# GLAD-RUC/FastEGNN

Measured on NVIDIA B200. Metric: layer fwd+bwd edges/sec (full train step: fwd+MSE+MMD+bwd+Adam), Water-3D shape, higher is better.
Workload: dtype tf32: tcgen05 TF32 operand tiles with fp32 accumulation and tanh.approx SiLU in the edge and virtual phases (fp16 operands with power-of-two scales in the edge backward), TF32 tiles in the node-side backward, error-compensated 3xTF32 tiles (fp32-grade) in the node-side forward, fp32 FMA in the per-g

## Files before the change

### fastegnn_b200/csrc/api.cu

```cuda
#include <cstdarg>
#include <cstdio>
#include <cstdlib>
#include <cstring>

#include "common.cuh"
#include "adam.cu"
#include "edge_kernels.cu"
#include "edge_tc.cu"
#include "edge_tc_bwd.cu"
#include "edge_tc_bwd2.cu"
#include "edge_tc_bwd3.cu"
#include "edge_tc_bwd4.cu"
#include "graph_kernels.cu"
#include "graph_prep.cu"
#include "radius_graph.cu"
#include "halo.cu"
#include "mmd.cu"
#include "node_kernels.cu"
#include "virtual_kernels.cu"
#include "virtual_tc.cu"
#include "node_tc.cu"
#include "dense_tc.cu"
#include "segment.cu"
#include "peak_probe.cu"
// ... 29 lines not shown
#define TRY(expr)            \
  do {                       \
    int rc__ = (expr);       \
    if (rc__ != 0) return rc__; \
  } while (0)

int g_edge_fwd_mode = 1;
int g_edge_bwd_mode = 6;

int g_virt_fwd_mode = 1;
int g_virt_bwd_mode = 1;
int g_node_fwd_mode = 3;
const bool g_node_pre_tc3 = getenv("FEGNN_NODE_PRE_TC3") == nullptr || atoi(getenv("FEGNN_NODE_PRE_TC3")) != 0;
int g_node_bwd_mode = 2;
int g_det = 0;
constexpr int kNodeTcMinN = 0;
inline bool node_bwd_tc(int N) { return g_node_bwd_mode == 1 || (g_node_bwd_mode == 2 && N >= kNodeTcMinN); }

int sm_count() {
  static int sms[64] = {};
  int dev = 0;
  if (cudaGetDevice(&dev) != cudaSuccess || dev < 0 || dev >= 64) return 148;
  if (sms[dev] == 0) {
    if (cudaDeviceGetAttribute(&sms[dev], cudaDevAttrMultiProcessorCount, dev) != cudaSuccess || sms[dev] <= 0) sms[dev] = 148;
  }
  return sms[dev];
}

int check_loss_ws(int N, int B, const float* ws, size_t floats) {
  if (!g_det) return 0;
// ... 126 lines not shown
  atomicAdd(gvnf + k * C + c, acc);
}
__global__ void final_gx_kernel(int N, const float* __restrict__ gx, const float* __restrict__ gxsum,
                                const int* __restrict__ batch, float* __restrict__ out) {
  int idx = blockIdx.x * blockDim.x + threadIdx.x;
  if (idx >= N * 3) return;
  int i = idx / 3, k = idx - i * 3;
  out[idx] = gx[idx] + gxsum[batch[i] * 3 + k];
}

}

namespace {

struct SideStream {
  cudaStream_t st = nullptr;
  cudaEvent_t fork = nullptr, join = nullptr, aux = nullptr;
};
SideStream* side_stream() {
  static SideStream per_dev[64];
  int dev = 0;
  if (cudaGetDevice(&dev) != cudaSuccess || dev < 0 || dev >= 64) return nullptr;
  SideStream* s = &per_dev[dev];
  if (s->st == nullptr) {
    if (cudaStreamCreateWithFlags(&s->st, cudaStreamNonBlocking) != cudaSuccess) return nullptr;
    if (cudaEventCreateWithFlags(&s->fork, cudaEventDisableTiming) != cudaSuccess) return nullptr;
    if (cudaEventCreateWithFlags(&s->join, cudaEventDisableTiming) != cudaSuccess) return nullptr;
    if (cudaEventCreateWithFlags(&s->aux, cudaEventDisableTiming) != cudaSuccess) return nullptr;
  }
  return s;
}
#define FORK(side, main)                                 \
  do {                                                   \
    CK(cudaEventRecord((side)->fork, (main)));           \
    CK(cudaStreamWaitEvent((side)->st, (side)->fork, 0)); \
  } while (0)
#define JOIN(side, main)                                 \
  do {                                                   \
    CK(cudaEventRecord((side)->join, (side)->st));       \
    CK(cudaStreamWaitEvent((main), (side)->join, 0));    \
  } while (0)

}
// ... 21 lines not shown
    if (mode != 0 && mode != 1 && !(mode == 2 && !fwd) && !(mode == 3 && fwd))
      return fail(FEGNN_EINVAL, "%s mode must be 0 or 1%s", phase, fwd ? " or 3 (3xTF32 phi_h)" : " or 2 (auto)");
    (fwd ? g_node_fwd_mode : g_node_bwd_mode) = mode;
    return 0;
  }
  if (strcmp(phase, "virtual_forward") == 0 || strcmp(phase, "virtual_backward") == 0) {
    if (mode != 0 && mode != 1) return fail(FEGNN_EINVAL, "%s mode must be 0 or 1", phase);
    (phase[8] == 'f' ? g_virt_fwd_mode : g_virt_bwd_mode) = mode;
    return 0;
  }
  if (strcmp(phase, "deterministic") == 0) {
    if (mode != 0 && mode != 1) return fail(FEGNN_EINVAL, "deterministic mode must be 0 or 1");
    g_det = mode;
    return 0;
  }
  return fail(FEGNN_EINVAL, "unknown phase '%s'", phase);
}
int fegnn_get_mode(const char* phase) {
  if (phase != nullptr && strcmp(phase, "edge_forward") == 0) return g_edge_fwd_mode;
  if (phase != nullptr && strcmp(phase, "edge_backward") == 0) return g_edge_bwd_mode;
  if (phase != nullptr && strcmp(phase, "node_forward") == 0) return g_node_fwd_mode;
  if (phase != nullptr && strcmp(phase, "node_backward") == 0) return g_node_bwd_mode;
  if (phase != nullptr && strcmp(phase, "virtual_forward") == 0) return g_virt_fwd_mode;
  if (phase != nullptr && strcmp(phase, "virtual_backward") == 0) return g_virt_bwd_mode;
  if (phase != nullptr && strcmp(phase, "deterministic") == 0) return g_det;
  return -1;
}

size_t fegnn_graph_prep_workspace_bytes(int32_t N, int32_t E) { return graph_prep_workspace_bytes(N, E); }

int fegnn_graph_prep(int32_t N, int32_t E, int32_t B, int32_t Fe, const int64_t* edge_index, const int64_t* data_batch,
                     const float* edge_attr, int32_t* perm, int32_t* rowptr, int32_t* row, int32_t* col,
                     int32_t* batch, int32_t* gptr, float* edge_attr_sorted, float* dinv, float* inv_nb,
                     void* workspace, size_t workspace_bytes, void* stream) {
  RQ(N >= 0 && E >= 0 && B >= 0 && Fe >= 0);
  RQ(rowptr && gptr && (N == 0 || (batch && data_batch && dinv)) && (B == 0 || inv_nb));
  RQ(E == 0 || (edge_index && perm && row && col && workspace));
  RQ(E == 0 || Fe == 0 || (edge_attr && edge_attr_sorted));
  if (workspace_bytes < graph_prep_workspace_bytes(N, E))
    return fail(FEGNN_ENOMEM, "graph_prep workspace %zu < %zu bytes", workspace_bytes, graph_prep_workspace_bytes(N, E));
// ... 225 lines not shown
    CK(launch_dense_bwd_tc(t2, sm_count(), S(stream)));
    return 0;
  }
  CK(launch_node_h_bwd(a, sm_count(), S(stream)));
  return 0;
}

int fegnn_virtual_backward(const fegnn_dims* d, const fegnn_graph* g, const fegnn_layer_params* p,
                           fegnn_layer_grads* gr, const float* x, const float* v, const float* Z,
                           const fegnn_layer_saved* sv, const float* gx_new, const float* gxsum_next,
                           const float* gDsum, const float* gUsum, const float* gu, float* gAv, float* gG1, float* gx,
                           float* gZ, float* gsv, float* gsg, float* gt, void* stream) {
  return fegnn_virtual_backward_inputs(d, g, p, gr, x, v, Z, sv, gx_new, gxsum_next, gDsum, gUsum, gu, gAv, gG1, gx, gZ, gsv,
                                       gsg, gt, nullptr, stream);
}
int fegnn_virtual_backward_inputs(const fegnn_dims* d, const fegnn_graph* g, const fegnn_layer_params* p,
                                  fegnn_layer_grads* gr, const float* x, const float* v, const float* Z,
                                  const fegnn_layer_saved* sv, const float* gx_new, const float* gxsum_next,
                                  const float* gDsum, const float* gUsum, const float* gu, float* gAv, float* gG1, float* gx,
                                  float* gZ, float* gsv, float* gsg, float* gt, const fegnn_input_grads* ig, void* stream) {
  NO_DET("the layer kernels add edge, node and graph sums across CTAs with float atomics");
  TRY(check_dims(d));
  TRY(check_flags_params(d, p));
  TRY(check_input_grads(d, ig));
  RQ(g && gr && x && v && Z && sv && gx_new && gDsum && gAv && gG1 && gx && gZ && gsv && gt);
  RQ(!(d->flags & FEGNN_F_GRAVITY) || gsg);
  VirtArgs a = virt_args(d, g, p, x, v, Z, sv);
  a.gx_new = gx_new; a.gxsum_next = gxsum_next; a.gDsum = gDsum; a.gUsum = gUsum; a.gu = gu;
  a.gAv = gAv; a.gG1 = gG1; a.gx = gx; a.gZ = gZ; a.gsv = gsv; a.gsg = gsg; a.gt = gt;
  a.g_wv1 = gr->edgev_w0; a.g_V2 = gr->edgev_w2; a.g_c2 = gr->edgev_b2;
  a.g_Wxv = gr->crv_w0; a.g_bxv = gr->crv_b0; a.g_wxv = gr->crv_w2;
  a.g_WX = gr->cvv_w0; a.g_bX = gr->cvv_b0; a.g_wX = gr->cvv_w2;
  a.g_wav = gr->attv_w; a.g_bav = gr->attv_b;
  if (!(d->flags & FEGNN_F_PREZEROED)) CK(zero_pair(gG1, kH * d->C * (size_t)d->B, gx, 3 * (size_t)d->Nl, S(stream)));
  if (d->flags & FEGNN_F_LAST) a.gu = nullptr;
  if (g_virt_bwd_mode == 1 && !(d->flags & FEGNN_F_ATTENTION) && gu != nullptr) {
    a.gu_work = const_cast<float*>(gu);
    a.u = sv->u;
    a.stats = reinterpret_cast<unsigned*>(sv->scratch);
    CK(launch_virtual_bwd_tc<4>(a, sm_count(), S(stream)));
  } else {
    CK(launch_virtual_bwd(a, sm_count(), S(stream)));
  }
  if (ig != nullptr && ig->node_vel != nullptr)
    CK(launch_input_grad_vel(d->N, sv->sv, gx_new, gxsum_next, g->batch, ig->node_vel, S(stream)));
  return 0;
}

int fegnn_edge_backward(const fegnn_dims* d, const fegnn_graph* g, const fegnn_layer_params* p, fegnn_layer_grads* gr,
                        const float* x, const fegnn_layer_saved* sv, const float* gm, const float* gt, float* gP,
                        float* gQ, float* gx, void* stream) {
  return fegnn_edge_backward_inputs(d, g, p, gr, x, sv, gm, gt, gP, gQ, gx, nullptr, stream);
}
int fegnn_edge_backward_inputs(const fegnn_dims* d, const fegnn_graph* g, const fegnn_layer_params* p, fegnn_layer_grads* gr,
                               const float* x, const fegnn_layer_saved* sv, const float* gm, const float* gt, float* gP,
                               float* gQ, float* gx, const fegnn_input_grads* ig, void* stream) {
  NO_DET("the layer kernels add edge, node and graph sums across CTAs with float atomics");
  TRY(check_dims(d));
  TRY(check_flags_params(d, p));
  TRY(check_input_grads(d, ig));
  RQ(g && gr && x && sv && gt && gP && gQ && gx);
  EdgeArgs a = edge_args(d, g, p, x, sv);
  a.gm = gm; a.gt = gt; a.gP = gP; a.gQ = gQ; a.gx = gx;
  a.g_w1 = gr->edge_w0; a.g_W2 = gr->edge_w2; a.g_b2 = gr->edge_b2;
  a.g_W3 = gr->cr_w0; a.g_b3 = gr->cr_b0; a.g_w4 = gr->cr_w2; a.g_wa = gr->att_w; a.g_ba = gr->att_b;
  const bool zero = !(d->flags & FEGNN_F_PREZEROED);
  if (zero) CK(zero_pair(gP, kH * (size_t)d->N, gQ, kH * (size_t)d->Nl, S(stream)));
  const bool tc_ok = d->Fe <= kTcMaxFe && !(d->flags & FEGNN_F_ATTENTION);
  int mode = g_edge_bwd_mode;
  if (mode == 6) mode = (tc_ok && sv->scratch != nullptr) ? 7 : 4;
  if ((mode == 7 || mode == 8) && (!tc_ok || sv->scratch == nullptr)) mode = 4;
  const bool pre = !(d->flags & FEGNN_F_STATS_READY);
  if (ig != nullptr && ig->edge_attr != nullptr) {
    a.g_ea = ig->edge_attr;
    a.perm = ig->perm;
    if (tc_ok && sv->scratch != nullptr && mode == 7) {
      CK((launch_edge_bwd_tc4<2, true>(a, reinterpret_cast<unsigned*>(sv->scratch), sm_count(), S(stream), zero && pre, pre)));
    } else {
      CK(launch_edge_bwd<true>(a, sm_count(), S(stream)));
    }
    return 0;
  }
  if (mode == 7) CK(launch_edge_bwd_tc4<2>(a, reinterpret_cast<unsigned*>(sv->scratch), sm_count(), S(stream), zero && pre, pre));
  else if (mode == 8) CK(launch_edge_bwd_tc4<4>(a, reinterpret_cast<unsigned*>(sv->scratch), sm_count(), S(stream), zero && pre, pre));
  else if (mode == 5 && tc_ok && sv->scratch != nullptr)
    CK(launch_edge_bwd_tc3(a, reinterpret_cast<unsigned*>(sv->scratch), sm_count(), S(stream), zero));
  else if (mode == 2 && tc_ok) CK(launch_edge_bwd_tc2<2>(a, sm_count(), S(stream)));
  else if ((mode == 4 || mode == 5) && tc_ok) CK(launch_edge_bwd_tc2<4>(a, sm_count(), S(stream)));
  else if (mode == 1 && tc_ok) CK(launch_edge_bwd_tc(a, sm_count(), S(stream)));
  else CK(launch_edge_bwd(a, sm_count(), S(stream)));
  return 0;
}

int fegnn_graph_pre_backward(const fegnn_dims* d, const fegnn_graph* g, const fegnn_layer_params* p,
                             fegnn_layer_grads* gr, const float* Sf, const fegnn_layer_saved* sv, const float* gG1,
                             float* gS, float* gZ, float* gxsum, void* stream) {
  NO_DET("the layer kernels add edge, node and graph sums across CTAs with float atomics");
  TRY(check_dims(d));
  RQ(g && p && gr && Sf && sv && gG1 && gS && gZ && gxsum);
  GraphArgs a = graph_args(d, g, p);
  a.S = Sf; a.M = sv->M; a.Zc = sv->Zc; a.gG1 = gG1; a.gS = gS; a.gZ = gZ; a.gxsum = gxsum;
  a.g_wv1 = gr->edgev_w0;
  CK(launch_graph_pre_bwd(a, S(stream)));
  return 0;
}

// ... 183 lines not shown
  const size_t N = d->N, Nl = d->Nl, B = d->B, C = d->C;
  float* p = base;
  auto take = [&](size_t n) { float* r = p; p += al4(n); return r; };
  for (int l = 0; l <= L; ++l) w->xsum[l] = take(B * 3);
  for (int l = 0; l <= L; ++l) {
    w->h[l] = take(N * kH); w->x[l] = take(Nl * 3); w->Z[l] = take(B * 3 * C); w->Sx[l] = take(B * C * kH);
  }
  for (int l = 0; l < L; ++l) {
    fegnn_layer_saved_bind(d, p, &w->saved[l]);
    p += fegnn_layer_saved_floats(d);
  }
}

struct BwdScratch {
  float *gh, *gx[2], *gZ[2], *gS[2], *gxsum[2], *gDsum, *gUsum, *gzh1, *gm, *gu, *gAv, *gG1[2], *gsv, *gsg, *gt, *gP[2], *gQ[2];
  size_t set_a_floats, set_b_floats;
};
size_t bwd_scratch_floats(const fegnn_dims* d) {
  const size_t N = d->N, Nl = d->Nl, B = d->B, C = d->C;
  return al4(N * kH) + 2 * al4(Nl * 3) + 2 * al4(B * 3 * C) + 2 * al4(B * C * kH) + 2 * al4(B * 3) + al4(B * 3 * C) +
         al4(B * C * kH) + 2 * al4(N * kH) + al4(N * C * kH) + al4(N * kH) + 2 * al4(B * C * kH) + 2 * al4(N) +
         al4(N * 3) + 2 * (al4(N * kH) + al4(Nl * kH));
}
void bwd_scratch_bind(const fegnn_dims* d, float* base, BwdScratch* s) {
  const size_t N = d->N, Nl = d->Nl, B = d->B, C = d->C;
  float* p = base;
  auto take = [&](size_t n) { float* r = p; p += al4(n); return r; };
  s->gh = take(N * kH);
  for (int k = 0; k < 2; ++k) { s->gG1[k] = take(B * C * kH); s->gx[k] = take(Nl * 3); }
  s->set_a_floats = al4(B * C * kH) + Nl * 3;
  s->gZ[0] = take(B * 3 * C); s->gZ[1] = take(B * 3 * C);
  s->gS[0] = take(B * C * kH); s->gS[1] = take(B * C * kH);
  s->gxsum[0] = take(B * 3); s->gxsum[1] = take(B * 3);
  s->gDsum = take(B * 3 * C); s->gUsum = take(B * C * kH);
  s->gzh1 = take(N * kH); s->gm = take(N * kH); s->gu = take(N * C * kH);
  s->gAv = take(N * kH);
  s->gsv = take(N); s->gsg = take(N); s->gt = take(N * 3);
  for (int k = 0; k < 2; ++k) { s->gP[k] = take(N * kH); s->gQ[k] = take(Nl * kH); }
  s->set_b_floats = al4(N * kH) + Nl * kH;
}

}

extern "C" {

size_t fegnn_model_workspace_floats(const fegnn_dims* d, int32_t L) { return model_ws_floats(d, L); }
size_t fegnn_model_backward_scratch_floats(const fegnn_dims* d) { return bwd_scratch_floats(d); }

int fegnn_model_forward(const fegnn_dims* d, int32_t L, int32_t Fin, const fegnn_graph* g,
                        const fegnn_layer_params* layers, const float* embed_w, const float* embed_b,
                        const float* vnf, const float* node_feat, const float* x0, const float* v,
                        const float* loc_mean, float* x_out, float* Z_out, float* workspace, size_t workspace_floats,
                        void* stream) {
  NO_DET("the layer kernels add edge, node and graph sums across CTAs with float atomics");
// ... 225 lines not shown
    dl.flags |= FEGNN_F_PREZEROED;
    const bool last = rf || l == L - 1;
    if (last) dl.flags |= FEGNN_F_LAST;
    const fegnn_layer_params* p = &layers[l];
    fegnn_layer_grads* gr = &grads[l];
    const fegnn_layer_saved* sv = &w.saved[l];
    const int ls = rf ? 0 : l;
    static const bool stats_fused = getenv("FEGNN_STATS_FUSED") == nullptr || atoi(getenv("FEGNN_STATS_FUSED")) != 0;
    if (stats_fused && !rf && g_virt_bwd_mode == 1 && !(d->flags & FEGNN_F_ATTENTION) && sv->scratch != nullptr &&
        (last || (node_bwd_tc(d->N) && dense_bwd_uses_rows(d->N, sm_count()))))
      dl.flags |= FEGNN_F_STATS_READY;
    TRY(fegnn_graph_post_backward(&dl, g, p, gr, w.Sx[ls], sv, gZ_new, gS_new, s.gZ[cur], s.gS[cur], s.gDsum, s.gUsum,
                                  side));
    if (!last) TRY(fegnn_node_h_backward(&dl, g, p, gr, sv, s.gh, s.gzh1, s.gm, s.gu, stream));
    JOIN(sd, st);
    TRY(fegnn_virtual_backward_inputs(&dl, g, p, gr, w.x[l], v, w.Z[l], sv, gx_new, gxsum_next, s.gDsum,
                                      last ? nullptr : s.gUsum, s.gu, s.gAv, s.gG1[cur], s.gx[cur], s.gZ[cur],
                                      s.gsv, s.gsg, s.gt, ig, stream));
    FORK(sd, st);
    TRY(fegnn_graph_pre_backward(&dl, g, p, gr, w.Sx[ls], sv, s.gG1[cur], s.gS[cur], s.gZ[cur], s.gxsum[cur], side));
    if (l > 0) {
      CK(cudaMemsetAsync(s.gG1[cur ^ 1], 0, sizeof(float) * s.set_a_floats, S(side)));
      CK(cudaMemsetAsync(s.gP[cur ^ 1], 0, sizeof(float) * s.set_b_floats, S(side)));
    }
    TRY(fegnn_edge_backward_inputs(&dl, g, p, gr, w.x[l], sv, last ? nullptr : s.gm, s.gt, s.gP[cur], s.gQ[cur], s.gx[cur],
                                   ig, stream));
    if (rf) TRY(fegnn_rf_vel_backward(d->N, v, p, gr, s.gsv, stream));
    TRY(fegnn_node_pre_backward_inputs(&dl, p, gr, w.h[ls], s.gP[cur], s.gQ[cur], s.gAv, last ? nullptr : s.gzh1, s.gsv, s.gsg,
                                       s.gh, ig, stream));
    gx_new = s.gx[cur]; gZ_new = s.gZ[cur]; gS_new = s.gS[cur]; gxsum_next = s.gxsum[cur];
    cur ^= 1;
  }
  FORK(sd, st);
  if (N > 0) {
    final_gx_kernel<<<(unsigned)((N * 3 + 255) / 256), 256, 0, S(side)>>>(d->N, gx_new, gxsum_next, g->batch, g_x0); ++g_launches;
    CK(cudaGetLastError());
  }
  CK(cudaMemcpyAsync(g_loc_mean, gZ_new, sizeof(float) * 3 * C * B, cudaMemcpyDeviceToDevice, S(side)));
  if (B > 0) {
    reduce_gS_kernel<<<(unsigned)((C * kH + 255) / 256), 256, 0, S(side)>>>(d->B, d->C, gS_new, g_vnf); ++g_launches;
    CK(cudaGetLastError());
// ... 83 lines not shown
```

### fastegnn_b200/csrc/edge_tc_bwd4.cu

```cuda
#include "common.cuh"
#include "umma.cuh"
#include <cuda_fp16.h>

namespace fegnn {
namespace bwd4 {

using bwd2::elect_one;
using bwd2::tmem_ld;
using bwd2::tmem_st_wait;
using bwd3::desc_add;
using bwd3::gemm_ts_k;
using bwd3::gemm_ts_mn;
using bwd3::gemm_wgrad;
using bwd3::h_chunk_off;
using bwd3::idesc_f16;
using bwd3::kTileBytes;
using bwd3::kWBytes;
using bwd3::make_desc_h;
using bwd3::pack2;
using bwd3::unpack2;

__device__ __forceinline__ uint32_t h2u(__half2 h) { return *reinterpret_cast<uint32_t*>(&h); }
__device__ __forceinline__ __half2 u2h(uint32_t u) { return *reinterpret_cast<__half2*>(&u); }
__device__ __forceinline__ __half2 tanh_h2(__half2 x) {
// ... 66 lines not shown
  float w4f[kH], wqf[kH];
  unsigned mw[2];
  uint32_t tmem_slot;
};
struct Geo {
  int srow[kTM], scol[kTM];
  float sq[kTM], snrm[kTM], sd[kTM * 3], sgte[kTM * 3], sgs[kTM], sea[kTM * kTcMaxFe];
};
template <int CG>
struct GroupVec {
  Geo geo[2];
  int irow[kTM], icol[kTM];
  float iea[kTM * kTcMaxFe];
  float spart[CG * kTM], sgqp[CG * kTM], ss[kTM];
  uint64_t bar[6];
};
__device__ __forceinline__ void cp_async4(void* dst, const void* src) {
  asm volatile("cp.async.ca.shared.global [%0], [%1], 4;" :: "r"(umma::smem_u32(dst)), "l"(src) : "memory");
}
__device__ __forceinline__ void cp_async_wait_all() { asm volatile("cp.async.wait_all;" ::: "memory"); }
template <int CG>
struct Smem4 {
  static constexpr int off_W2 = 0, off_W3 = kWBytes;
  static constexpr int off_groups = 2 * kWBytes;
  static constexpr int g_TA = 0, g_TM = kTileBytes, g_AUX = 2 * kTileBytes, g_TG = 3 * kTileBytes, g_T3 = 4 * kTileBytes;
  static constexpr int g_vec = 5 * kTileBytes;
  static constexpr int g_bytes = ((g_vec + (int)sizeof(GroupVec<CG>) + 1023) / 1024) * 1024;
  static constexpr int off_svec = off_groups + 2 * g_bytes;
  static constexpr size_t bytes = off_svec + sizeof(SharedVec) + 1024;
};
constexpr uint32_t kACC = 0, kOPA = 64, kD2T = 96, kD1T = 128, kGroupCols = 160;
constexpr uint32_t kR3 = 320, kR2 = 392, kDXZ = 464, kDW4 = 472;

__device__ __forceinline__ float pow2_to(float bound, int e_target) {
  if (!(bound > 0.f) || !(bound < 3.0e38f)) return 1.f;
  int e;
  frexpf(bound, &e);
  e = e_target - e;
  e = e < -60 ? -60 : (e > 60 ? 60 : e);
  return ldexpf(1.f, e);
}

template <int CG, bool kEa>
__global__ void __launch_bounds__(256 * CG, 1) edge_bwd_tc4_kernel(EdgeArgs a, const unsigned* stats) {
  VTR_DECL();
  constexpr int NTG = 128 * CG, NT = 2 * NTG, CPT = kH / CG, NP = CPT / 2, NWG = NTG / 32, RPW = kTM / NWG;
  using SM = Smem4<CG>;
  using GV = GroupVec<CG>;
  extern __shared__ uint8_t smem_raw[];
  uint8_t* smem = smem_raw + ((1024u - (umma::smem_u32(smem_raw) & 1023u)) & 1023u);
  SharedVec* sv = reinterpret_cast<SharedVec*>(smem + SM::off_svec);
  const int t = threadIdx.x, G = t / NTG, tg = t - G * NTG, wg = tg >> 5, lane = t & 31;
  const int quarter = wg & 3, cg = wg >> 2, row = quarter * 32 + lane, c0 = cg * CPT;
  uint8_t* gs = smem + SM::off_groups + G * SM::g_bytes;
  GV* v = reinterpret_cast<GV*>(gs + SM::g_vec);
  uint8_t *TA = gs + SM::g_TA, *TM = gs + SM::g_TM, *AUX = gs + SM::g_AUX, *TG = gs + SM::g_TG, *T3 = gs + SM::g_T3;
  const bool use_tanh = a.flags & FEGNN_F_TANH, norm = a.flags & FEGNN_F_NORMALIZE;
  auto group_sync = [&]() { asm volatile("bar.sync %0, %1;" :: "r"(1 + G), "n"(NTG) : "memory"); };
  pdl_trigger();
// ... 85 lines not shown
  const float k32 = s2 / s3, k21 = s1 / s2;
  const float r3 = 1.f / s3, r2 = 1.f / s2, r1 = 1.f / s1, ra = 1.f / sa, rdot = 1.f / sdot, rq = 1.f / (s1 * swq);
  const uint32_t tbase = tmem + G * kGroupCols;
  const uint32_t tlane = tbase + ((uint32_t)(quarter * 32) << 16);
  const uint32_t twg = tmem + ((uint32_t)(16 * G) << 16);
  const uint32_t id_k = idesc_f16(128, 64, 0, 0), id_mn = idesc_f16(128, 64, 0, 1);
  const uint32_t id_wg72 = idesc_f16(64, 72, 1, 1), id_aux = idesc_f16(64, 8, 1, 1);
  const uint64_t dW2k = make_desc_h(umma::smem_u32(smem + SM::off_W2), 16), dW3k = make_desc_h(umma::smem_u32(smem + SM::off_W3), 16);
  const uint64_t dW2m = make_desc_h(umma::smem_u32(smem + SM::off_W2), kWBytes), dW3m = make_desc_h(umma::smem_u32(smem + SM::off_W3), kWBytes);
  const uint64_t dTG = make_desc_h(umma::smem_u32(TG), kTileBytes);
  const uint64_t dTM_AUX = make_desc_h(umma::smem_u32(TM), kTileBytes);
  const uint64_t dTA_AUX = make_desc_h(umma::smem_u32(TA), 2 * kTileBytes);
  const uint64_t dTMa = make_desc_h(umma::smem_u32(TM), kTileBytes);
  const uint64_t dT3a = make_desc_h(umma::smem_u32(T3), kTileBytes);
  const uint64_t dAUX = make_desc_h(umma::smem_u32(AUX), kTileBytes);
  uint32_t phase = 0;
  bool first_tile = true;
  const int l16 = lane & 15, hsel = lane >> 4;

  const int ntiles = (a.E + kTM - 1) / kTM, tstride = gridDim.x * 2;
  auto load_idx_async = [&](int tl) {
    const int e = tl * kTM + tg;
    if (e < a.E) {
      cp_async4(&v->irow[tg], a.row + e);
      cp_async4(&v->icol[tg], a.col + e);
      for (int f = 0; f < a.Fe; ++f) cp_async4(&v->iea[tg * kTcMaxFe + f], a.ea + (size_t)e * a.Fe + f);
    } else {
      v->irow[tg] = -1;
    }
  };
  auto geometry = [&](Geo* gg) {
    cp_async_wait_all();
    const int r = v->irow[tg];
    int c = 0;
    float d0 = 0, d1 = 0, d2 = 0, q = 0, nrm = 1.f, g0 = 0, g1 = 0, g2 = 0;
// ... 14 lines not shown
#pragma unroll
    for (int f = 0; f < kTcMaxFe; ++f) gg->sea[tg * kTcMaxFe + f] = ea[f];
    gg->sd[tg * 3 + 0] = d0; gg->sd[tg * 3 + 1] = d1; gg->sd[tg * 3 + 2] = d2;
    if (norm) {
      nrm = sqrtf(q) + a.eps;
      const float inv = 1.f / nrm;
      d0 *= inv; d1 *= inv; d2 *= inv;
    }
    gg->srow[tg] = r;
    gg->scol[tg] = c;
    gg->sq[tg] = q;
    gg->snrm[tg] = nrm;
    gg->sgte[tg * 3 + 0] = g0; gg->sgte[tg * 3 + 1] = g1; gg->sgte[tg * 3 + 2] = g2;
    gg->sgs[tg] = d0 * g0 + d1 * g1 + d2 * g2;
  };
  int cur = 0;
  if (tg < kTM && blockIdx.x * 2 + G < ntiles) {
    load_idx_async(blockIdx.x * 2 + G);
    geometry(&v->geo[0]);
    if (blockIdx.x * 2 + G + tstride < ntiles) load_idx_async(blockIdx.x * 2 + G + tstride);
  }
  for (int tile = blockIdx.x * 2 + G; tile < ntiles; tile += tstride, cur ^= 1) {
    const Geo* geo = &v->geo[cur];
    if (!first_tile) {
      umma::mbar_wait(&v->bar[4], phase ^ 1);
    VTR();
      umma::fence_after();
    }
    umma::fence_before();
    group_sync();
    VTR();
    if (tg < kTM)
      *reinterpret_cast<uint4*>(AUX + h_chunk_off(tg, 0)) =
          make_uint4(pack2(geo->srow[tg] >= 0 ? 1.f : 0.f, geo->sq[tg]), pack2(geo->sea[tg * kTcMaxFe], geo->sea[tg * kTcMaxFe + 1]),
                     pack2(geo->sea[tg * kTcMaxFe + 2], geo->sea[tg * kTcMaxFe + 3]), 0u);
    group_sync();
    VTR();
    {
// ... 51 lines not shown
      tmem_stu<NP>(tlane + kD1T + cg * NP, pd);
      tmem_st_wait();
    }
    umma::fence_smem_to_async();
    umma::fence_before();
    group_sync();
    VTR();
    if (wg == 0) {
      umma::fence_after();
      if (elect_one()) {
        gemm_ts_k(tbase + kACC, tbase + kOPA, dW2k, id_k);
        umma::commit(&v->bar[0]);
      }
      __syncwarp();
    }
    if (tg < kTM && tile + tstride < ntiles) {
      geometry(&v->geo[cur ^ 1]);
      if (tile + 2 * tstride < ntiles) load_idx_async(tile + 2 * tstride);
    }
    umma::mbar_wait(&v->bar[0], phase);
    VTR();
    umma::fence_after();
    {
      float z[CPT];
      uint32_t pm[NP], pd[NP];
      tmem_ld<CPT>(tlane + kACC + c0, z);
#pragma unroll
      for (int j = 0; j < CPT; j += 4) {
        const float4 hb = *reinterpret_cast<const float4*>(sv->hb2 + c0 + j);
        __half2 a0, e0, a1v, e1;
        silu_grad_h2(__floats2half2_rn(fmaf(z[j], 0.5f, hb.x), fmaf(z[j + 1], 0.5f, hb.y)), a0, e0);
        silu_grad_h2(__floats2half2_rn(fmaf(z[j + 2], 0.5f, hb.z), fmaf(z[j + 3], 0.5f, hb.w)), a1v, e1);
        pm[j >> 1] = h2u(a0); pm[(j >> 1) + 1] = h2u(a1v);
// ... 172 lines not shown
        }
      }
    }
    umma::fence_smem_to_async();
    umma::fence_before();
    group_sync();
    VTR();
    if (wg == 0) {
      umma::fence_after();
      if (elect_one()) {
        gemm_wgrad(twg + kDXZ, dTMa, dAUX, id_aux, !first_tile);
        umma::commit(&v->bar[4]);
      }
      __syncwarp();
    }
    phase ^= 1;
    first_tile = false;
    if (!(a.exp & 3u)) {
      constexpr int RH = RPW / 2;
      int rk[RH + 1], ck[RH];
      uint2 uu[RH];
#pragma unroll
      for (int i = 0; i < RH; ++i) {
        const int rr = wg * RPW + hsel * RH + i;
        rk[i] = geo->srow[rr];
        ck[i] = geo->scol[rr];
        uu[i] = *reinterpret_cast<const uint2*>(TM + h_chunk_off(rr, l16 >> 1) + ((l16 & 1) << 3));
      }
      rk[RH] = -2;
      float4 run = make_float4(0.f, 0.f, 0.f, 0.f);
#pragma unroll
// ... 25 lines not shown
#pragma unroll
      for (int o = 1; o < 32; o <<= 1) {
        const int ku = __shfl_up_sync(0xffffffffu, r, o);
        const float u0 = __shfl_up_sync(0xffffffffu, gd[0], o), u1 = __shfl_up_sync(0xffffffffu, gd[1], o),
                    u2 = __shfl_up_sync(0xffffffffu, gd[2], o);
        if (lane >= o && ku == r) { gd[0] += u0; gd[1] += u1; gd[2] += u2; }
      }
      const int kd = __shfl_down_sync(0xffffffffu, r, 1);
      if ((lane == 31 || kd != r) && r >= 0) {
#pragma unroll
        for (int k = 0; k < 3; ++k) atomicAdd(a.gx + (size_t)r * 3 + k, gd[k]);
      }
    }
    if constexpr (kEa) {
      if (tg < kTM && geo->srow[tg] >= 0) {
        const int e = tile * kTM + tg;
        float* dst = a.g_ea + (size_t)(a.perm != nullptr ? a.perm[e] : e) * a.Fe;
        for (int f = 0; f < a.Fe; ++f) {
          float ge = 0.f;
#pragma unroll
          for (int g = 0; g < CG; ++g) ge += reinterpret_cast<const float*>(T3)[(f * CG + g) * kTM + tg];
          dst[f] += ge * (2.f * r1);
        }
      }
    }
    VTR();
  }
  if (!first_tile) umma::mbar_wait(&v->bar[4], phase ^ 1);
    VTR();
  umma::fence_after();
  umma::fence_before();
  __syncthreads();
    VTR();
  umma::fence_after();
  const bool has0 = blockIdx.x * 2 + 0 < ntiles, has1 = blockIdx.x * 2 + 1 < ntiles;
  if (G == 0) {
    const int n = quarter * 16 + (lane & 15);
    const bool mine = (lane < 16) ? has0 : has1;
    const uint32_t tl = tmem + ((uint32_t)(quarter * 32) << 16);
    float w[CPT];
    auto flush_rows = [&](float* base, const float (&w)[CPT], float r) {
      if (!mine || base == nullptr) return;
      float* dst = base + (size_t)n * kH + c0;
      if ((reinterpret_cast<uintptr_t>(dst) & 15) == 0) {
#pragma unroll
        for (int j = 0; j < CPT; j += 4)
          atomicAdd(reinterpret_cast<float4*>(dst + j), make_float4(w[j] * r, w[j + 1] * r, w[j + 2] * r, w[j + 3] * r));
      } else {
#pragma unroll
        for (int j = 0; j < CPT; ++j) atomicAdd(dst + j, w[j] * r);
// ... 21 lines not shown
      }
    }
  }
  umma::fence_before();
  __syncthreads();
    VTR();
  if (t < 32) umma::tmem_dealloc<512>(tmem);
  VTR();
  VTR_PRINT("edge_bwd");
}

}

template <int CG, bool kEa = false>
inline cudaError_t launch_edge_bwd_tc4(const EdgeArgs& a, unsigned* stats, int sms, cudaStream_t st, bool zero_stats = true,
                                       bool run_stats = true) {
  static DevOnce attr;
  const size_t bytes = bwd4::Smem4<CG>::bytes;
  if (!attr.get()) {
    cudaError_t e = cudaFuncSetAttribute(bwd4::edge_bwd_tc4_kernel<CG, kEa>, cudaFuncAttributeMaxDynamicSharedMemorySize, (int)bytes);
    if (e != cudaSuccess) return e;
    attr.set();
  }
  const int ntiles = (a.E + kTM - 1) / kTM;
  if (ntiles == 0) return cudaSuccess;
  const int pairs = (ntiles + 1) / 2;
  const int grid = pairs < sms ? pairs : sms;
  cudaError_t e = zero_stats ? cudaMemsetAsync(stats, 0, 4 * sizeof(unsigned), st) : cudaSuccess;
  if (e != cudaSuccess) return e;
  int sblocks = (int)(((size_t)a.N * kH + 256 * 4 - 1) / (256 * 4));
  sblocks = sblocks < 1 ? 1 : (sblocks > sms ? sms : sblocks);
  if (run_stats) {
    e = launch_pdl(bwd3::edge_bwd_stats_kernel, sblocks, 256, 0, st, a.N, a.Nl, a.x, a.gt, a.gm, stats);
    if (e != cudaSuccess) return e;
  }
  e = launch_pdl(bwd4::edge_bwd_tc4_kernel<CG, kEa>, grid, 256 * CG, bytes, st, a, (const unsigned*)stats);
  if (e != cudaSuccess) return e;
  return cudaGetLastError();
}

}
```

### fastegnn_b200/csrc/virtual_tc.cu

```cuda
#include "common.cuh"
#include "umma.cuh"
#include <cuda_fp16.h>

namespace fegnn {
namespace vtc {

using bwd2::desc_advance;
using bwd2::gemm_ts_kmajor;
using bwd2::gemm_ts_mn;
using bwd2::gemm_wgrad;
using bwd2::idesc_tf32;
using bwd2::make_desc_mn;
using bwd2::mma_ts;
using bwd2::mn_chunk_off;
using bwd2::mn_load_row;
using bwd2::mn_store_row;
using bwd2::silu_grad_tc;
using bwd2::tmem_ld;
using bwd2::tmem_st;
using bwd2::tmem_st_wait;

__device__ __forceinline__ float silu_tc(float z) {
  const float t = 0.5f * z;
  float th;
// ... 685 lines not shown
    }
    cp_async_wait();
    __syncthreads();
    VTR();
    if (single && warp == NW - 1) small_from_rows(v->g.sgD, &v->acc, C, TN, lane);
    if (t < TN) {
      const int i = tile * TN + t;
      if (i < a.N) {
        const float di = a.dinv != nullptr ? a.dinv[i] : 1.f;
        float gsv = 0.f, gsg = 0.f;
#pragma unroll
        for (int k = 0; k < 3; ++k) {
          const float g = v->g.sgxn[t * 3 + k];
          float sum = 0.f;
          for (int c = 0; c < C; ++c) sum += v->g.sgD[(t * C + c) * 3 + k];
          a.gx[(size_t)i * 3 + k] = g - sum;
          a.gt[(size_t)i * 3 + k] = g * di;
          if (a.stats != nullptr) {
            st_gt = fmaxf(st_gt, fabsf(g * di));
            st_x = fmaxf(st_x, fabsf(a.x[(size_t)i * 3 + k] - a.x[k]));
          }
          gsv = fmaf(g, a.v[(size_t)i * 3 + k], gsv);
          gsg = fmaf(g, a.grav[k], gsg);
        }
        a.gsv[i] = gsv;
        if (grav) a.gsg[i] = gsg;
      }
    }
    umma::mbar_wait(&v->bar[1], phase);
    VTR();
    umma::fence_after();
    {
// ... 369 lines not shown
          if (!single) atomicAdd(a.gZ + ((size_t)b * 3 + k) * C + c, gD[k]);
        }
      }
      v->g.sgD[t * 3 + 0] = gD[0]; v->g.sgD[t * 3 + 1] = gD[1]; v->g.sgD[t * 3 + 2] = gD[2];
    }
    __syncthreads();
    VTR();
    if (single && warp == NW - 1) small_from_rows(v->g.sgD, &v->acc, C, TN, lane);
    if (t < TN) {
      const int i = tile * TN + t;
      if (i < a.N) {
#pragma unroll
        for (int k = 0; k < 3; ++k) {
          float sum = 0.f;
          for (int c = 0; c < C; ++c) sum += v->g.sgD[(t * C + c) * 3 + k];
          a.gx[(size_t)i * 3 + k] -= sum;
        }
      }
    }
  }
  acc_flush<NT>(&v->acc, cur_b, C, a.gG1, a.gZ, nullptr);
  if (!first_tile) umma::mbar_wait(&v->bar[2], phase ^ 1);
    VTR();
  umma::fence_after();
  if (!first_tile) {
    const int n = quarter * 16 + lane;
    float w[CPT];
    tmem_ld<CPT>(tlane + kT_R2 + 32, w);
    if (lane < 16 && a.g_V2 != nullptr) {
      float* dst = a.g_V2 + (size_t)n * kH + c0;
      if ((reinterpret_cast<uintptr_t>(dst) & 15) == 0) {
// ... 34 lines not shown
    if (e != cudaSuccess) return e;
    attr.set();
  }
  const int TN = kTM / a.C;
  const int ntiles = (a.N + TN - 1) / TN;
  if (ntiles == 0) return cudaSuccess;
  const int grid = ntiles < 2 * sms ? ntiles : 2 * sms;
  if (cudaError_t e_ = launch_pdl(vtc::virtual_fwd_tc_kernel<CG>, grid, 128 * CG, bytes, st, a)) return e_;
  return cudaGetLastError();
}

}

namespace fegnn {
template <int CG>
cudaError_t launch_virtual_bwd_tc(const VirtArgs& a, int sms, cudaStream_t st) {
  static DevOnce attr;
  if (!attr.get()) {
    cudaError_t e = cudaFuncSetAttribute(vtc::virtual_bwd_heads_tc_kernel<CG>, cudaFuncAttributeMaxDynamicSharedMemorySize,
                                         (int)vtc::HeadsSmem::bytes);
    if (e != cudaSuccess) return e;
    e = cudaFuncSetAttribute(vtc::virtual_bwd_trunk_tc_kernel<CG>, cudaFuncAttributeMaxDynamicSharedMemorySize,
                             (int)vtc::TrunkSmem::bytes);
    if (e != cudaSuccess) return e;
    attr.set();
  }
  const int TN = kTM / a.C;
  const int ntiles = (a.N + TN - 1) / TN;
  if (ntiles == 0) return cudaSuccess;
  const int grid = ntiles < sms ? ntiles : sms;
  if (cudaError_t e_ = launch_pdl(vtc::virtual_bwd_heads_tc_kernel<CG>, grid, 128 * CG, vtc::HeadsSmem::bytes, st, a)) return e_;
  cudaError_t e = cudaGetLastError();
  if (e != cudaSuccess) return e;
  if (cudaError_t e_ = launch_pdl(vtc::virtual_bwd_trunk_tc_kernel<CG>, grid, 128 * CG, vtc::TrunkSmem::bytes, st, a)) return e_;
  return cudaGetLastError();
}
}
```

Baseline: 787.6 million.

## Overlap virtual backward with edge backward on split SMs via side stream

Adds a per-layer mode that computes the gt gradient and its stats in a small standalone kernel first. The virtual backward then runs on a separate stream capped at a subset of SMs, while the edge backward runs concurrently on the remaining SMs. The edge backward kernel gains an atomic tile-claim work queue so its CTAs can balance dynamically when sharing the GPU. The virtual kernels switch to atomic adds into gx when running concurrently. This trades extra atomics, an extra launch and heuristic SM partitioning (fixed 2.9 weight) for concurrency between two phases that each underfill the machine.

```diff
diff --git a/fastegnn_b200/csrc/api.cu b/fastegnn_b200/csrc/api.cu
--- a/fastegnn_b200/csrc/api.cu
+++ b/fastegnn_b200/csrc/api.cu
@@ -67,6 +67,8 @@
 const bool g_node_pre_tc3 = getenv("FEGNN_NODE_PRE_TC3") == nullptr || atoi(getenv("FEGNN_NODE_PRE_TC3")) != 0;
 int g_node_bwd_mode = 2;
 int g_det = 0;
+int g_layer_overlap = getenv("FEGNN_LAYER_OVERLAP") ? atoi(getenv("FEGNN_LAYER_OVERLAP")) : 1;
+const int g_overlap_vsms = getenv("FEGNN_OVERLAP_VSMS") ? atoi(getenv("FEGNN_OVERLAP_VSMS")) : 0;
 constexpr int kNodeTcMinN = 0;
 inline bool node_bwd_tc(int N) { return g_node_bwd_mode == 1 || (g_node_bwd_mode == 2 && N >= kNodeTcMinN); }
 
@@ -223,8 +225,8 @@
 namespace {
 
 struct SideStream {
-  cudaStream_t st = nullptr;
-  cudaEvent_t fork = nullptr, join = nullptr, aux = nullptr;
+  cudaStream_t st = nullptr, vst = nullptr;
+  cudaEvent_t fork = nullptr, join = nullptr, aux = nullptr, vfork = nullptr, vjoin = nullptr;
 };
 SideStream* side_stream() {
   static SideStream per_dev[64];
@@ -236,6 +238,9 @@
     if (cudaEventCreateWithFlags(&s->fork, cudaEventDisableTiming) != cudaSuccess) return nullptr;
     if (cudaEventCreateWithFlags(&s->join, cudaEventDisableTiming) != cudaSuccess) return nullptr;
     if (cudaEventCreateWithFlags(&s->aux, cudaEventDisableTiming) != cudaSuccess) return nullptr;
+    if (cudaStreamCreateWithFlags(&s->vst, cudaStreamNonBlocking) != cudaSuccess) return nullptr;
+    if (cudaEventCreateWithFlags(&s->vfork, cudaEventDisableTiming) != cudaSuccess) return nullptr;
+    if (cudaEventCreateWithFlags(&s->vjoin, cudaEventDisableTiming) != cudaSuccess) return nullptr;
   }
   return s;
 }
@@ -287,6 +292,11 @@
     g_det = mode;
     return 0;
   }
+  if (strcmp(phase, "layer_overlap") == 0) {
+    if (mode < 0 || mode > 2) return fail(FEGNN_EINVAL, "layer_overlap mode must be 0, 1 (auto) or 2");
+    g_layer_overlap = mode;
+    return 0;
+  }
   return fail(FEGNN_EINVAL, "unknown phase '%s'", phase);
 }
 int fegnn_get_mode(const char* phase) {
@@ -297,6 +307,7 @@
   if (phase != nullptr && strcmp(phase, "virtual_forward") == 0) return g_virt_fwd_mode;
   if (phase != nullptr && strcmp(phase, "virtual_backward") == 0) return g_virt_bwd_mode;
   if (phase != nullptr && strcmp(phase, "deterministic") == 0) return g_det;
+  if (phase != nullptr && strcmp(phase, "layer_overlap") == 0) return g_layer_overlap;
   return -1;
 }
 
@@ -552,16 +563,21 @@
   return fegnn_virtual_backward_inputs(d, g, p, gr, x, v, Z, sv, gx_new, gxsum_next, gDsum, gUsum, gu, gAv, gG1, gx, gZ, gsv,
                                        gsg, gt, nullptr, stream);
 }
-int fegnn_virtual_backward_inputs(const fegnn_dims* d, const fegnn_graph* g, const fegnn_layer_params* p,
-                                  fegnn_layer_grads* gr, const float* x, const float* v, const float* Z,
-                                  const fegnn_layer_saved* sv, const float* gx_new, const float* gxsum_next,
-                                  const float* gDsum, const float* gUsum, const float* gu, float* gAv, float* gG1, float* gx,
-                                  float* gZ, float* gsv, float* gsg, float* gt, const fegnn_input_grads* ig, void* stream) {
+static bool virt_bwd_tc(const fegnn_dims* d, const float* gu) {
+  return g_virt_bwd_mode == 1 && !(d->flags & FEGNN_F_ATTENTION) && gu != nullptr;
+}
+static int virtual_backward_run(const fegnn_dims* d, const fegnn_graph* g, const fegnn_layer_params* p,
+                                fegnn_layer_grads* gr, const float* x, const float* v, const float* Z,
+                                const fegnn_layer_saved* sv, const float* gx_new, const float* gxsum_next,
+                                const float* gDsum, const float* gUsum, const float* gu, float* gAv, float* gG1, float* gx,
+                                float* gZ, float* gsv, float* gsg, float* gt, const fegnn_input_grads* ig, bool gt_ahead,
+                                int cap, void* stream) {
   NO_DET("the layer kernels add edge, node and graph sums across CTAs with float atomics");
   TRY(check_dims(d));
   TRY(check_flags_params(d, p));
   TRY(check_input_grads(d, ig));
   RQ(g && gr && x && v && Z && sv && gx_new && gDsum && gAv && gG1 && gx && gZ && gsv && gt);
+  RQ(!gt_ahead || virt_bwd_tc(d, gu));
   RQ(!(d->flags & FEGNN_F_GRAVITY) || gsg);
   VirtArgs a = virt_args(d, g, p, x, v, Z, sv);
   a.gx_new = gx_new; a.gxsum_next = gxsum_next; a.gDsum = gDsum; a.gUsum = gUsum; a.gu = gu;
@@ -572,17 +588,26 @@
   a.g_wav = gr->attv_w; a.g_bav = gr->attv_b;
   if (!(d->flags & FEGNN_F_PREZEROED)) CK(zero_pair(gG1, kH * d->C * (size_t)d->B, gx, 3 * (size_t)d->Nl, S(stream)));
   if (d->flags & FEGNN_F_LAST) a.gu = nullptr;
-  if (g_virt_bwd_mode == 1 && !(d->flags & FEGNN_F_ATTENTION) && gu != nullptr) {
+  if (virt_bwd_tc(d, gu)) {
     a.gu_work = const_cast<float*>(gu);
     a.u = sv->u;
     a.stats = reinterpret_cast<unsigned*>(sv->scratch);
-    CK(launch_virtual_bwd_tc<4>(a, sm_count(), S(stream)));
+    if (gt_ahead) { a.gt = nullptr; a.stats = nullptr; }
+    CK(launch_virtual_bwd_tc<4>(a, cap, S(stream)));
   } else {
     CK(launch_virtual_bwd(a, sm_count(), S(stream)));
   }
   if (ig != nullptr && ig->node_vel != nullptr)
     CK(launch_input_grad_vel(d->N, sv->sv, gx_new, gxsum_next, g->batch, ig->node_vel, S(stream)));
   return 0;
+}
+int fegnn_virtual_backward_inputs(const fegnn_dims* d, const fegnn_graph* g, const fegnn_layer_params* p,
+                                  fegnn_layer_grads* gr, const float* x, const float* v, const float* Z,
+                                  const fegnn_layer_saved* sv, const float* gx_new, const float* gxsum_next,
+                                  const float* gDsum, const float* gUsum, const float* gu, float* gAv, float* gG1, float* gx,
+                                  float* gZ, float* gsv, float* gsg, float* gt, const fegnn_input_grads* ig, void* stream) {
+  return virtual_backward_run(d, g, p, gr, x, v, Z, sv, gx_new, gxsum_next, gDsum, gUsum, gu, gAv, gG1, gx, gZ, gsv, gsg, gt,
+                              ig, false, sm_count(), stream);
 }
 
 int fegnn_edge_backward(const fegnn_dims* d, const fegnn_graph* g, const fegnn_layer_params* p, fegnn_layer_grads* gr,
@@ -590,9 +615,9 @@
                         float* gQ, float* gx, void* stream) {
   return fegnn_edge_backward_inputs(d, g, p, gr, x, sv, gm, gt, gP, gQ, gx, nullptr, stream);
 }
-int fegnn_edge_backward_inputs(const fegnn_dims* d, const fegnn_graph* g, const fegnn_layer_params* p, fegnn_layer_grads* gr,
-                               const float* x, const fegnn_layer_saved* sv, const float* gm, const float* gt, float* gP,
-                               float* gQ, float* gx, const fegnn_input_grads* ig, void* stream) {
+static int edge_backward_run(const fegnn_dims* d, const fegnn_graph* g, const fegnn_layer_params* p, fegnn_layer_grads* gr,
+                             const float* x, const fegnn_layer_saved* sv, const float* gm, const float* gt, float* gP,
+                             float* gQ, float* gx, const fegnn_input_grads* ig, unsigned* claim, int cap, void* stream) {
   NO_DET("the layer kernels add edge, node and graph sums across CTAs with float atomics");
   TRY(check_dims(d));
   TRY(check_flags_params(d, p));
@@ -613,14 +638,14 @@
     a.g_ea = ig->edge_attr;
     a.perm = ig->perm;
     if (tc_ok && sv->scratch != nullptr && mode == 7) {
-      CK((launch_edge_bwd_tc4<2, true>(a, reinterpret_cast<unsigned*>(sv->scratch), sm_count(), S(stream), zero && pre, pre)));
+      CK((launch_edge_bwd_tc4<2, true>(a, reinterpret_cast<unsigned*>(sv->scratch), cap, S(stream), zero && pre, pre, claim)));
     } else {
       CK(launch_edge_bwd<true>(a, sm_count(), S(stream)));
     }
     return 0;
   }
-  if (mode == 7) CK(launch_edge_bwd_tc4<2>(a, reinterpret_cast<unsigned*>(sv->scratch), sm_count(), S(stream), zero && pre, pre));
-  else if (mode == 8) CK(launch_edge_bwd_tc4<4>(a, reinterpret_cast<unsigned*>(sv->scratch), sm_count(), S(stream), zero && pre, pre));
+  if (mode == 7) CK(launch_edge_bwd_tc4<2>(a, reinterpret_cast<unsigned*>(sv->scratch), cap, S(stream), zero && pre, pre, claim));
+  else if (mode == 8) CK(launch_edge_bwd_tc4<4>(a, reinterpret_cast<unsigned*>(sv->scratch), cap, S(stream), zero && pre, pre, claim));
   else if (mode == 5 && tc_ok && sv->scratch != nullptr)
     CK(launch_edge_bwd_tc3(a, reinterpret_cast<unsigned*>(sv->scratch), sm_count(), S(stream), zero));
   else if (mode == 2 && tc_ok) CK(launch_edge_bwd_tc2<2>(a, sm_count(), S(stream)));
@@ -628,6 +653,11 @@
   else if (mode == 1 && tc_ok) CK(launch_edge_bwd_tc(a, sm_count(), S(stream)));
   else CK(launch_edge_bwd(a, sm_count(), S(stream)));
   return 0;
+}
+int fegnn_edge_backward_inputs(const fegnn_dims* d, const fegnn_graph* g, const fegnn_layer_params* p, fegnn_layer_grads* gr,
+                               const float* x, const fegnn_layer_saved* sv, const float* gm, const float* gt, float* gP,
+                               float* gQ, float* gx, const fegnn_input_grads* ig, void* stream) {
+  return edge_backward_run(d, g, p, gr, x, sv, gm, gt, gP, gQ, gx, ig, nullptr, sm_count(), stream);
 }
 
 int fegnn_graph_pre_backward(const fegnn_dims* d, const fegnn_graph* g, const fegnn_layer_params* p,
@@ -841,13 +871,14 @@
 
 struct BwdScratch {
   float *gh, *gx[2], *gZ[2], *gS[2], *gxsum[2], *gDsum, *gUsum, *gzh1, *gm, *gu, *gAv, *gG1[2], *gsv, *gsg, *gt, *gP[2], *gQ[2];
+  unsigned* claim[2];
   size_t set_a_floats, set_b_floats;
 };
 size_t bwd_scratch_floats(const fegnn_dims* d) {
   const size_t N = d->N, Nl = d->Nl, B = d->B, C = d->C;
   return al4(N * kH) + 2 * al4(Nl * 3) + 2 * al4(B * 3 * C) + 2 * al4(B * C * kH) + 2 * al4(B * 3) + al4(B * 3 * C) +
          al4(B * C * kH) + 2 * al4(N * kH) + al4(N * C * kH) + al4(N * kH) + 2 * al4(B * C * kH) + 2 * al4(N) +
-         al4(N * 3) + 2 * (al4(N * kH) + al4(Nl * kH));
+         al4(N * 3) + 2 * (al4(N * kH) + al4(Nl * kH) + 4);
 }
 void bwd_scratch_bind(const fegnn_dims* d, float* base, BwdScratch* s) {
   const size_t N = d->N, Nl = d->Nl, B = d->B, C = d->C;
@@ -863,8 +894,10 @@
   s->gzh1 = take(N * kH); s->gm = take(N * kH); s->gu = take(N * C * kH);
   s->gAv = take(N * kH);
   s->gsv = take(N); s->gsg = take(N); s->gt = take(N * 3);
-  for (int k = 0; k < 2; ++k) { s->gP[k] = take(N * kH); s->gQ[k] = take(Nl * kH); }
-  s->set_b_floats = al4(N * kH) + Nl * kH;
+  for (int k = 0; k < 2; ++k) {
+    s->gP[k] = take(N * kH); s->gQ[k] = take(Nl * kH); s->claim[k] = reinterpret_cast<unsigned*>(take(4));
+  }
+  s->set_b_floats = al4(N * kH) + al4(Nl * kH) + 4;
 }
 
 }
@@ -1120,17 +1153,39 @@
                                   side));
     if (!last) TRY(fegnn_node_h_backward(&dl, g, p, gr, sv, s.gh, s.gzh1, s.gm, s.gu, stream));
     JOIN(sd, st);
-    TRY(fegnn_virtual_backward_inputs(&dl, g, p, gr, w.x[l], v, w.Z[l], sv, gx_new, gxsum_next, s.gDsum,
-                                      last ? nullptr : s.gUsum, s.gu, s.gAv, s.gG1[cur], s.gx[cur], s.gZ[cur],
-                                      s.gsv, s.gsg, s.gt, ig, stream));
-    FORK(sd, st);
+    const int vtiles = (d->N + kTM / d->C - 1) / (kTM / d->C);
+    const bool overlap = virt_bwd_tc(&dl, s.gu) &&
+                         (g_layer_overlap == 2 || (g_layer_overlap == 1 && vtiles > sm_count() && 2 * vtiles <= 3 * sm_count()));
+    void* vstream = overlap ? static_cast<void*>(sd->vst) : stream;
+    int vsms = g_overlap_vsms;
+    if (overlap && vsms <= 0) {
+      const double wv = 2.9 * vtiles, we = (double)((d->E + kTM - 1) / kTM);
+      vsms = (int)(sm_count() * wv / (wv + we) + 0.5);
+    }
+    vsms = min(max(vsms, 1), sm_count() - 1);
+    if (overlap) {
+      VirtArgs ga = virt_args(&dl, g, p, w.x[l], v, w.Z[l], sv);
+      ga.gx_new = gx_new; ga.gxsum_next = gxsum_next; ga.gt = s.gt;
+      CK(launch_virtual_bwd_gt(ga, reinterpret_cast<unsigned*>(sv->scratch), st));
+      CK(cudaEventRecord(sd->vfork, st));
+      CK(cudaStreamWaitEvent(sd->vst, sd->vfork, 0));
+    }
+    TRY(virtual_backward_run(&dl, g, p, gr, w.x[l], v, w.Z[l], sv, gx_new, gxsum_next, s.gDsum, last ? nullptr : s.gUsum, s.gu,
+                             s.gAv, s.gG1[cur], s.gx[cur], s.gZ[cur], s.gsv, s.gsg, s.gt, ig, overlap,
+                             overlap ? vsms : sm_count(), vstream));
+    CK(cudaEventRecord(sd->fork, S(vstream)));
+    CK(cudaStreamWaitEvent(sd->st, sd->fork, 0));
     TRY(fegnn_graph_pre_backward(&dl, g, p, gr, w.Sx[ls], sv, s.gG1[cur], s.gS[cur], s.gZ[cur], s.gxsum[cur], side));
     if (l > 0) {
       CK(cudaMemsetAsync(s.gG1[cur ^ 1], 0, sizeof(float) * s.set_a_floats, S(side)));
       CK(cudaMemsetAsync(s.gP[cur ^ 1], 0, sizeof(float) * s.set_b_floats, S(side)));
     }
-    TRY(fegnn_edge_backward_inputs(&dl, g, p, gr, w.x[l], sv, last ? nullptr : s.gm, s.gt, s.gP[cur], s.gQ[cur], s.gx[cur],
-                                   ig, stream));
+    TRY(edge_backward_run(&dl, g, p, gr, w.x[l], sv, last ? nullptr : s.gm, s.gt, s.gP[cur], s.gQ[cur], s.gx[cur], ig,
+                          overlap ? s.claim[cur] : nullptr, overlap ? sm_count() - vsms : sm_count(), stream));
+    if (overlap) {
+      CK(cudaEventRecord(sd->vjoin, sd->vst));
+      CK(cudaStreamWaitEvent(st, sd->vjoin, 0));
+    }
     if (rf) TRY(fegnn_rf_vel_backward(d->N, v, p, gr, s.gsv, stream));
     TRY(fegnn_node_pre_backward_inputs(&dl, p, gr, w.h[ls], s.gP[cur], s.gQ[cur], s.gAv, last ? nullptr : s.gzh1, s.gsv, s.gsg,
                                        s.gh, ig, stream));
diff --git a/fastegnn_b200/csrc/edge_tc_bwd4.cu b/fastegnn_b200/csrc/edge_tc_bwd4.cu
--- a/fastegnn_b200/csrc/edge_tc_bwd4.cu
+++ b/fastegnn_b200/csrc/edge_tc_bwd4.cu
@@ -104,6 +104,8 @@
   float iea[kTM * kTcMaxFe];
   float spart[CG * kTM], sgqp[CG * kTM], ss[kTM];
   uint64_t bar[6];
+  int qt[4];
+  int had;
 };
 __device__ __forceinline__ void cp_async4(void* dst, const void* src) {
   asm volatile("cp.async.ca.shared.global [%0], [%1], 4;" :: "r"(umma::smem_u32(dst)), "l"(src) : "memory");
@@ -132,7 +134,7 @@
 }
 
 template <int CG, bool kEa>
-__global__ void __launch_bounds__(256 * CG, 1) edge_bwd_tc4_kernel(EdgeArgs a, const unsigned* stats) {
+__global__ void __launch_bounds__(256 * CG, 1) edge_bwd_tc4_kernel(EdgeArgs a, const unsigned* stats, unsigned* claim) {
   VTR_DECL();
   constexpr int NTG = 128 * CG, NT = 2 * NTG, CPT = kH / CG, NP = CPT / 2, NWG = NTG / 32, RPW = kTM / NWG;
   using SM = Smem4<CG>;
@@ -248,11 +250,11 @@
   const uint64_t dTMa = make_desc_h(umma::smem_u32(TM), kTileBytes);
   const uint64_t dT3a = make_desc_h(umma::smem_u32(T3), kTileBytes);
   const uint64_t dAUX = make_desc_h(umma::smem_u32(AUX), kTileBytes);
-  uint32_t phase = 0;
   bool first_tile = true;
   const int l16 = lane & 15, hsel = lane >> 4;
 
-  const int ntiles = (a.E + kTM - 1) / kTM, tstride = gridDim.x * 2;
+  const int ntiles = (a.E + kTM - 1) / kTM;
+  auto claim_tile = [&](int prev) { return claim != nullptr ? (int)atomicAdd(claim, 1u) : prev + (int)gridDim.x * 2; };
   auto load_idx_async = [&](int tl) {
     const int e = tl * kTM + tg;
     if (e < a.E) {
@@ -297,14 +299,21 @@
     gg->sgte[tg * 3 + 0] = g0; gg->sgte[tg * 3 + 1] = g1; gg->sgte[tg * 3 + 2] = g2;
     gg->sgs[tg] = d0 * g0 + d1 * g1 + d2 * g2;
   };
-  int cur = 0;
-  if (tg < kTM && blockIdx.x * 2 + G < ntiles) {
-    load_idx_async(blockIdx.x * 2 + G);
+  if (tg == 0) {
+    v->qt[0] = claim != nullptr ? (int)atomicAdd(claim, 1u) : (int)blockIdx.x * 2 + G;
+    v->qt[1] = claim_tile(v->qt[0]);
+  }
+  group_sync();
+  if (tg < kTM && v->qt[0] < ntiles) {
+    load_idx_async(v->qt[0]);
     geometry(&v->geo[0]);
-    if (blockIdx.x * 2 + G + tstride < ntiles) load_idx_async(blockIdx.x * 2 + G + tstride);
-  }
-  for (int tile = blockIdx.x * 2 + G; tile < ntiles; tile += tstride, cur ^= 1) {
-    const Geo* geo = &v->geo[cur];
+    if (v->qt[1] < ntiles) load_idx_async(v->qt[1]);
+  }
+  int k = 0;
+  for (; v->qt[k & 3] < ntiles; ++k) {
+    const uint32_t phase = k & 1;
+    const Geo* geo = &v->geo[k & 1];
+    if (tg == 0) v->qt[(k + 2) & 3] = claim_tile(v->qt[(k + 1) & 3]);
     if (!first_tile) {
       umma::mbar_wait(&v->bar[4], phase ^ 1);
     VTR();
@@ -386,9 +395,9 @@
       }
       __syncwarp();
     }
-    if (tg < kTM && tile + tstride < ntiles) {
-      geometry(&v->geo[cur ^ 1]);
-      if (tile + 2 * tstride < ntiles) load_idx_async(tile + 2 * tstride);
+    if (tg < kTM && v->qt[(k + 1) & 3] < ntiles) {
+      geometry(&v->geo[(k & 1) ^ 1]);
+      if (v->qt[(k + 2) & 3] < ntiles) load_idx_async(v->qt[(k + 2) & 3]);
     }
     umma::mbar_wait(&v->bar[0], phase);
     VTR();
@@ -591,7 +600,6 @@
       }
       __syncwarp();
     }
-    phase ^= 1;
     first_tile = false;
     if (!(a.exp & 3u)) {
       constexpr int RH = RPW / 2;
@@ -647,7 +655,7 @@
     }
     if constexpr (kEa) {
       if (tg < kTM && geo->srow[tg] >= 0) {
-        const int e = tile * kTM + tg;
+        const int e = v->qt[k & 3] * kTM + tg;
         float* dst = a.g_ea + (size_t)(a.perm != nullptr ? a.perm[e] : e) * a.Fe;
         for (int f = 0; f < a.Fe; ++f) {
           float ge = 0.f;
@@ -659,14 +667,16 @@
     }
     VTR();
   }
-  if (!first_tile) umma::mbar_wait(&v->bar[4], phase ^ 1);
-    VTR();
+  if (!first_tile) umma::mbar_wait(&v->bar[4], (k & 1) ^ 1);
+    VTR();
+  if (tg == 0) v->had = first_tile ? 0 : 1;
   umma::fence_after();
   umma::fence_before();
   __syncthreads();
     VTR();
   umma::fence_after();
-  const bool has0 = blockIdx.x * 2 + 0 < ntiles, has1 = blockIdx.x * 2 + 1 < ntiles;
+  const bool has0 = reinterpret_cast<const GV*>(smem + SM::off_groups + SM::g_vec)->had != 0;
+  const bool has1 = reinterpret_cast<const GV*>(smem + SM::off_groups + SM::g_bytes + SM::g_vec)->had != 0;
   if (G == 0) {
     const int n = quarter * 16 + (lane & 15);
     const bool mine = (lane < 16) ? has0 : has1;
@@ -718,7 +728,7 @@
 
 template <int CG, bool kEa = false>
 inline cudaError_t launch_edge_bwd_tc4(const EdgeArgs& a, unsigned* stats, int sms, cudaStream_t st, bool zero_stats = true,
-                                       bool run_stats = true) {
+                                       bool run_stats = true, unsigned* claim = nullptr) {
   static DevOnce attr;
   const size_t bytes = bwd4::Smem4<CG>::bytes;
   if (!attr.get()) {
@@ -738,7 +748,7 @@
     e = launch_pdl(bwd3::edge_bwd_stats_kernel, sblocks, 256, 0, st, a.N, a.Nl, a.x, a.gt, a.gm, stats);
     if (e != cudaSuccess) return e;
   }
-  e = launch_pdl(bwd4::edge_bwd_tc4_kernel<CG, kEa>, grid, 256 * CG, bytes, st, a, (const unsigned*)stats);
+  e = launch_pdl(bwd4::edge_bwd_tc4_kernel<CG, kEa>, grid, 256 * CG, bytes, st, a, (const unsigned*)stats, claim);
   if (e != cudaSuccess) return e;
   return cudaGetLastError();
 }
diff --git a/fastegnn_b200/csrc/virtual_tc.cu b/fastegnn_b200/csrc/virtual_tc.cu
--- a/fastegnn_b200/csrc/virtual_tc.cu
+++ b/fastegnn_b200/csrc/virtual_tc.cu
@@ -723,8 +723,12 @@
           const float g = v->g.sgxn[t * 3 + k];
           float sum = 0.f;
           for (int c = 0; c < C; ++c) sum += v->g.sgD[(t * C + c) * 3 + k];
-          a.gx[(size_t)i * 3 + k] = g - sum;
-          a.gt[(size_t)i * 3 + k] = g * di;
+          if (a.gt != nullptr) {
+            a.gx[(size_t)i * 3 + k] = g - sum;
+            a.gt[(size_t)i * 3 + k] = g * di;
+          } else {
+            atomicAdd(a.gx + (size_t)i * 3 + k, g - sum);
+          }
           if (a.stats != nullptr) {
             st_gt = fmaxf(st_gt, fabsf(g * di));
             st_x = fmaxf(st_x, fabsf(a.x[(size_t)i * 3 + k] - a.x[k]));
@@ -1124,7 +1128,8 @@
         for (int k = 0; k < 3; ++k) {
           float sum = 0.f;
           for (int c = 0; c < C; ++c) sum += v->g.sgD[(t * C + c) * 3 + k];
-          a.gx[(size_t)i * 3 + k] -= sum;
+          if (a.gt != nullptr) a.gx[(size_t)i * 3 + k] -= sum;
+          else atomicAdd(a.gx + (size_t)i * 3 + k, -sum);
         }
       }
     }
@@ -1189,7 +1194,7 @@
 
 namespace fegnn {
 template <int CG>
-cudaError_t launch_virtual_bwd_tc(const VirtArgs& a, int sms, cudaStream_t st) {
+cudaError_t launch_virtual_bwd_tc(const VirtArgs& a, int cap, cudaStream_t st) {
   static DevOnce attr;
   if (!attr.get()) {
     cudaError_t e = cudaFuncSetAttribute(vtc::virtual_bwd_heads_tc_kernel<CG>, cudaFuncAttributeMaxDynamicSharedMemorySize,
@@ -1203,11 +1208,51 @@
   const int TN = kTM / a.C;
   const int ntiles = (a.N + TN - 1) / TN;
   if (ntiles == 0) return cudaSuccess;
-  const int grid = ntiles < sms ? ntiles : sms;
+  const int grid = ntiles < cap ? ntiles : cap;
   if (cudaError_t e_ = launch_pdl(vtc::virtual_bwd_heads_tc_kernel<CG>, grid, 128 * CG, vtc::HeadsSmem::bytes, st, a)) return e_;
   cudaError_t e = cudaGetLastError();
   if (e != cudaSuccess) return e;
   if (cudaError_t e_ = launch_pdl(vtc::virtual_bwd_trunk_tc_kernel<CG>, grid, 128 * CG, vtc::TrunkSmem::bytes, st, a)) return e_;
   return cudaGetLastError();
 }
-}
+
+constexpr int kGtThreads = 256;
+__global__ void __launch_bounds__(kGtThreads) virtual_bwd_gt_kernel(int N, const float* __restrict__ x, const float* gx_new,
+                                                                   const float* gxsum_next, const int* __restrict__ batch,
+                                                                   const float* __restrict__ dinv, float* gt, unsigned* stats) {
+  __shared__ float red[2][kGtThreads / 32];
+  pdl_trigger();
+  pdl_wait();
+  const int idx = blockIdx.x * kGtThreads + threadIdx.x, lane = threadIdx.x & 31, warp = threadIdx.x >> 5;
+  float mg = 0.f, mx = 0.f;
+  if (idx < N * 3) {
+    const int i = idx / 3, k = idx - i * 3;
+    float g = gx_new[idx];
+    if (gxsum_next != nullptr) g += gxsum_next[batch[i] * 3 + k];
+    g *= dinv != nullptr ? dinv[i] : 1.f;
+    gt[idx] = g;
+    mg = fabsf(g);
+    mx = fabsf(x[idx] - x[k]);
+  }
+  if (stats == nullptr) return;
+#pragma unroll
+  for (int o = 16; o > 0; o >>= 1) {
+    mg = fmaxf(mg, __shfl_xor_sync(0xffffffffu, mg, o));
+    mx = fmaxf(mx, __shfl_xor_sync(0xffffffffu, mx, o));
+  }
+  if (lane == 0) { red[0][warp] = mg; red[1][warp] = mx; }
+  __syncthreads();
+  if (threadIdx.x == 0) {
+    for (int w = 1; w < kGtThreads / 32; ++w) { mg = fmaxf(mg, red[0][w]); mx = fmaxf(mx, red[1][w]); }
+    atomicMax(stats + 0, __float_as_uint(mg));
+    atomicMax(stats + 2, __float_as_uint(mx));
+  }
+}
+inline cudaError_t launch_virtual_bwd_gt(const VirtArgs& a, unsigned* stats, cudaStream_t st) {
+  if (a.N == 0) return cudaSuccess;
+  if (cudaError_t e = launch_pdl(virtual_bwd_gt_kernel, (a.N * 3 + kGtThreads - 1) / kGtThreads, kGtThreads, 0, st, a.N, a.x,
+                                 a.gx_new, a.gxsum_next, a.batch, a.dinv, a.gt, stats))
+    return e;
+  return cudaGetLastError();
+}
+}
```

After: 842.9 million, median of 6. 1.07x the previous value.
